# lijx10/USIP

Hardware: AMD Instinct MI355X
Metric: point-clouds/sec detector fwd+bwd (higher is better)
Workload: dtype f32 results; matrix-bound products emulated from 2 fp16 planes per operand (22-bit operands, 3 plane products, exact ...; 1 GPU; KITTI detector N=16384 M=512 K=64 batch=8 pairs/GPU (BASELINE configs[2]); detector=RPN_Detector_Ball, clouds_per_gpu=16, surface_normal_len=4, node_knn_k_1=16, ball_radius=2, ball_k=64, cloud=slab, matmul=f32x2, step=fwd+losses+bwd+adam, launch=HIP graph replay (ONE graph per step: forward, backward, Adam), parallelism=dp1

## Files before the change

### usip_amd/csrc/knn.hip

```cpp
#include "common.h"

namespace {

constexpr int CPL_MAX = 16;

template <int CPL>
__global__ __launch_bounds__(256) void knn_kernel(
    const float* __restrict__ query, const float* __restrict__ database, int32_t* __restrict__ out,
    int M, int N, int K)
{
    const int lane = threadIdx.x & 63;
    const int m = blockIdx.x * 4 + (threadIdx.x >> 6);
    const int b = blockIdx.y;
    if (m >= M) return;
    const float* qb = query + (long long)b * 3 * M;
    const float* db = database + (long long)b * 3 * N;
    const float qx = qb[m], qy = qb[M + m], qz = qb[2 * M + m];
    float d[CPL];
    unsigned taken = 0;
#pragma unroll
    for (int i = 0; i < CPL; ++i) {
        const int j = i * 64 + lane;
        d[i] = (j < N) ? usip_dist(qx, qy, qz, db[j], db[N + j], db[2 * N + j]) : __builtin_inff();
        if (!(d[i] == d[i])) d[i] = __builtin_inff();
        if (j >= N) taken |= 1u << i;
    }
    int32_t* o = out + ((long long)b * M + m) * K;
    for (int k = 0; k < K; ++k) {
        float best = __builtin_inff();
        int bj = 0x7fffffff;
#pragma unroll
        for (int i = 0; i < CPL; ++i) {
            const int j = i * 64 + lane;
            if (!((taken >> i) & 1u) && (bj == 0x7fffffff || d[i] < best)) { best = d[i]; bj = j; }
        }
        float wbest = best;
        int wj = bj;
#pragma unroll
        for (int off = 32; off > 0; off >>= 1) {
            const float ov = __shfl_xor(wbest, off);
            const int oj = __shfl_xor(wj, off);
            if (ov < wbest || (ov == wbest && oj < wj)) { wbest = ov; wj = oj; }
        }
        if (lane == 0) o[k] = (wj == 0x7fffffff) ? 0 : wj;
        if (wj != 0x7fffffff && (wj & 63) == lane) taken |= 1u << (wj >> 6);
    }
}

}

extern "C" int usip_knn_f32(const float* query, const float* database, int32_t* idx,
                            int B, int M, int N, int K, void* stream)
{
    if (B < 0 || M < 0 || N < 1 || K < 1 || K > N) return USIP_EINVAL;
    if ((long long)B * M == 0) return USIP_OK;
    if (!query || !database || !idx || B > 65535 || N > 64 * CPL_MAX) return USIP_EINVAL;
    const dim3 grid(usip_ceil_div(M, 4), B), block(256);
    if (N <= 256) USIP_LAUNCH(knn_kernel<4>, grid, block, 0, (hipStream_t)stream, query, database, idx, M, N, K);
    else if (N <= 512) USIP_LAUNCH(knn_kernel<8>, grid, block, 0, (hipStream_t)stream, query, database, idx, M, N, K);
    else USIP_LAUNCH(knn_kernel<16>, grid, block, 0, (hipStream_t)stream, query, database, idx, M, N, K);
    USIP_LAUNCH_CHECK();
    return USIP_OK;
}

namespace {

constexpr int KP_T = 256;
constexpr int KP_CAP = 1024;

__device__ __forceinline__ unsigned kp_wave_sorted_pick(unsigned v, int lane, int pick)
{
#pragma unroll
    for (int k = 2; k <= 64; k <<= 1)
#pragma unroll
        for (int j = k >> 1; j > 0; j >>= 1) {
            const unsigned o = __shfl_xor(v, j);
            const bool up = ((lane & k) == 0);
            const bool lower = ((lane & j) == 0);
            const unsigned mn = v < o ? v : o, mx = v < o ? o : v;
            v = (up == lower) ? mn : mx;
        }
    return __shfl(v, pick);
}

template <int J>
__global__ __launch_bounds__(KP_T) void knn_points_kernel(
    const float* __restrict__ node, const float* __restrict__ x, int32_t* __restrict__ out, int M, int N, int K)
{
    __shared__ unsigned long long cand[KP_CAP];
    __shared__ unsigned wtau[4];
    __shared__ unsigned wcnt[4];
    __shared__ unsigned ncand;

    const int tid = threadIdx.x, lane = tid & 63, wave = tid >> 6;
    const int m = blockIdx.x, b = blockIdx.y;
    const float* nb_ = node + (long long)b * 3 * M;
    const float* xb = x + (long long)b * 3 * N;
    const float qx = nb_[m], qy = nb_[M + m], qz = nb_[2 * M + m];

    unsigned d[J];
    unsigned tmin = 0xFFFFFFFFu;
#pragma unroll
    for (int j = 0; j < J; ++j) {
        const int n = j * KP_T + tid;
        unsigned key = 0xFFFFFFFFu;
        if (n < N) {
            const float v = usip_dist(qx, qy, qz, xb[n], xb[N + n], xb[2 * N + n]);
            key = __builtin_bit_cast(unsigned, v);
            if (!(v == v)) key = 0xFFC00000u;
        }
        d[j] = key;
        tmin = key < tmin ? key : tmin;
    }
    if (tid == 0) ncand = 0;
    const int q = (K + 3) >> 2;
    const unsigned tw = kp_wave_sorted_pick(tmin, lane, q - 1);
    if (lane == 0) wtau[wave] = tw;
    __syncthreads();
    unsigned tau = wtau[0];
#pragma unroll
    for (int w = 1; w < 4; ++w) tau = wtau[w] > tau ? wtau[w] : tau;

    auto compact = [&](unsigned long long bound) {
#pragma unroll
        for (int j = 0; j < J; ++j) {
            const int n = j * KP_T + tid;
            const unsigned long long k48 = ((unsigned long long)d[j] << 16) | (unsigned)n;
            if (n < N && k48 <= bound) {
                const unsigned slot = atomicAdd(&ncand, 1u);
                if (slot < (unsigned)KP_CAP) cand[slot] = k48;
            }
        }
    };
    compact(((unsigned long long)tau << 16) | 0xFFFFull);
    __syncthreads();
    unsigned c = ncand;
    if (c > (unsigned)KP_CAP) {
        unsigned long long lo = 0, hi = (1ull << 48) - 1;
        while (lo < hi) {
            const unsigned long long mid = lo + ((hi - lo) >> 1);
            unsigned cnt = 0;
#pragma unroll
            for (int j = 0; j < J; ++j) {
                const int n = j * KP_T + tid;
                const unsigned long long k48 = ((unsigned long long)d[j] << 16) | (unsigned)n;
                cnt += (n < N && k48 <= mid) ? 1u : 0u;
            }
#pragma unroll
            for (int off = 32; off > 0; off >>= 1) cnt += __shfl_xor(cnt, off);
            __syncthreads();
            if (lane == 0) wcnt[wave] = cnt;
            __syncthreads();
            const unsigned total = wcnt[0] + wcnt[1] + wcnt[2] + wcnt[3];
            if (total >= (unsigned)K) hi = mid; else lo = mid + 1;
        }
        __syncthreads();
        if (tid == 0) ncand = 0;
        __syncthreads();
        compact(lo);
        __syncthreads();
        c = ncand;
    }
    int32_t* o = out + ((long long)b * M + m) * K;
    for (unsigned i = tid; i < c; i += KP_T) {
        const unsigned long long mine = cand[i];
        unsigned rank = 0;
        for (unsigned t = 0; t < c; ++t) rank += (cand[t] < mine) ? 1u : 0u;
        if (rank < (unsigned)K) o[rank] = (int32_t)(mine & 0xFFFFull);
    }
}

}

extern "C" int usip_knn_points_f32(const float* node, const float* x, int32_t* idx, int B, int M, int N, int K,
                                   void* stream)
{
    if (B < 0 || M < 0 || N < 1 || K < 1 || K > N || K > 256 || N > 64 * KP_T) return USIP_EINVAL;
    if ((long long)B * M == 0) return USIP_OK;
    if (!node || !x || !idx || B > 65535) return USIP_EINVAL;
    hipStream_t st = (hipStream_t)stream;
    const dim3 grid((unsigned)M, (unsigned)B), block(KP_T);
    const int per = usip_ceil_div(N, KP_T);
    if (per <= 8) USIP_LAUNCH(knn_points_kernel<8>, grid, block, 0, st, node, x, idx, M, N, K);
    else if (per <= 16) USIP_LAUNCH(knn_points_kernel<16>, grid, block, 0, st, node, x, idx, M, N, K);
    else if (per <= 32) USIP_LAUNCH(knn_points_kernel<32>, grid, block, 0, st, node, x, idx, M, N, K);
    else USIP_LAUNCH(knn_points_kernel<64>, grid, block, 0, st, node, x, idx, M, N, K);
    USIP_LAUNCH_CHECK();
    return USIP_OK;
}
```

Measured before the change: 4000 point-clouds/s.

## Presort per-lane KNN candidates and use DPP wave-min for selection

The KNN kernel now packs each distance and index into a 64-bit key and bitonic-sorts each lane's CPL candidates in registers. Each of the K selection rounds then only inspects the lane's head element instead of rescanning all CPL values. The cross-lane argmin uses DPP row ops plus readlanes rather than a shuffle butterfly, and output indices are buffered in registers and written coalesced every 64 picks. The trade-off is extra register pressure from the 64-bit keys and the upfront sorting network.

```diff
diff --git a/usip_amd/csrc/knn.hip b/usip_amd/csrc/knn.hip
--- a/usip_amd/csrc/knn.hip
+++ b/usip_amd/csrc/knn.hip
@@ -3,6 +3,24 @@
 namespace {
 
 constexpr int CPL_MAX = 16;
+
+template <int CTRL>
+__device__ __forceinline__ unsigned knn_dpp_min(unsigned v)
+{
+    const unsigned o = (unsigned)__builtin_amdgcn_update_dpp(-1, (int)v, CTRL, 0xF, 0xF, false);
+    return o < v ? o : v;
+}
+
+__device__ __forceinline__ unsigned knn_wave_min(unsigned v)
+{
+    v = knn_dpp_min<0xB1>(v);
+    v = knn_dpp_min<0x4E>(v);
+    v = knn_dpp_min<0x141>(v);
+    v = knn_dpp_min<0x140>(v);
+    const unsigned r0 = (unsigned)__builtin_amdgcn_readlane((int)v, 0), r1 = (unsigned)__builtin_amdgcn_readlane((int)v, 16);
+    const unsigned r2 = (unsigned)__builtin_amdgcn_readlane((int)v, 32), r3 = (unsigned)__builtin_amdgcn_readlane((int)v, 48);
+    return min(min(r0, r1), min(r2, r3));
+}
 
 template <int CPL>
 __global__ __launch_bounds__(256) void knn_kernel(
@@ -16,34 +34,45 @@
     const float* qb = query + (long long)b * 3 * M;
     const float* db = database + (long long)b * 3 * N;
     const float qx = qb[m], qy = qb[M + m], qz = qb[2 * M + m];
-    float d[CPL];
-    unsigned taken = 0;
+    unsigned long long key[CPL];
 #pragma unroll
     for (int i = 0; i < CPL; ++i) {
         const int j = i * 64 + lane;
-        d[i] = (j < N) ? usip_dist(qx, qy, qz, db[j], db[N + j], db[2 * N + j]) : __builtin_inff();
-        if (!(d[i] == d[i])) d[i] = __builtin_inff();
-        if (j >= N) taken |= 1u << i;
-    }
+        float d = (j < N) ? usip_dist(qx, qy, qz, db[j], db[N + j], db[2 * N + j]) : __builtin_inff();
+        if (!(d == d)) d = __builtin_inff();
+        key[i] = (j < N) ? (((unsigned long long)__builtin_bit_cast(unsigned, d) << 32) | (unsigned)j) : ~0ull;
+    }
+#pragma unroll
+    for (int k = 2; k <= CPL; k <<= 1)
+#pragma unroll
+        for (int j = k >> 1; j > 0; j >>= 1)
+#pragma unroll
+            for (int i = 0; i < CPL; ++i) {
+                const int l = i ^ j;
+                if (l > i) {
+                    const unsigned long long x = key[i], y = key[l];
+                    const bool swap = ((i & k) == 0) ? (y < x) : (x < y);
+                    key[i] = swap ? y : x;
+                    key[l] = swap ? x : y;
+                }
+            }
     int32_t* o = out + ((long long)b * M + m) * K;
+    int32_t res = 0;
     for (int k = 0; k < K; ++k) {
-        float best = __builtin_inff();
-        int bj = 0x7fffffff;
-#pragma unroll
-        for (int i = 0; i < CPL; ++i) {
-            const int j = i * 64 + lane;
-            if (!((taken >> i) & 1u) && (bj == 0x7fffffff || d[i] < best)) { best = d[i]; bj = j; }
-        }
-        float wbest = best;
-        int wj = bj;
-#pragma unroll
-        for (int off = 32; off > 0; off >>= 1) {
-            const float ov = __shfl_xor(wbest, off);
-            const int oj = __shfl_xor(wj, off);
-            if (ov < wbest || (ov == wbest && oj < wj)) { wbest = ov; wj = oj; }
-        }
-        if (lane == 0) o[k] = (wj == 0x7fffffff) ? 0 : wj;
-        if (wj != 0x7fffffff && (wj & 63) == lane) taken |= 1u << (wj >> 6);
+        const unsigned hi = (unsigned)(key[0] >> 32), lo = (unsigned)key[0];
+        const unsigned dmin = knn_wave_min(hi);
+        const unsigned wj = knn_wave_min(hi == dmin ? lo : 0xffffffffu);
+        if (lane == (k & 63)) res = (wj == 0xffffffffu) ? 0 : (int32_t)wj;
+        if ((k & 63) == 63 || k == K - 1) {
+            const int kk = (k & ~63) + lane;
+            if (kk <= k) o[kk] = res;
+        }
+        const bool won = lo == wj;
+        if (won) {
+#pragma unroll
+            for (int i = 0; i + 1 < CPL; ++i) key[i] = key[i + 1];
+            key[CPL - 1] = ~0ull;
+        }
     }
 }
 
```

After: 4001 point-clouds/s (median of 2 runs). No clear change (+0.0%).
